# neozenith/sqlite-muninn

Measured on AMD Instinct MI355X. Metric: kNN queries/sec (10k-query batch, k=10, ef=128, 1M x 768 f32 HNSW index) + recall@10, higher is better.
Workload: dtype f32

## Files before the change

### sqlite-muninn_amd/csrc/mn_beam.hpp

```cpp
#pragma once
#include "mn_dist.hpp"

template <bool COH> DEVI int ld_link(const int *p) {
    if (COH)
        return __hip_atomic_load(p, __ATOMIC_RELAXED, __HIP_MEMORY_SCOPE_AGENT);
    return *p;
}
DEVI void st_link(int *p, int v) { __hip_atomic_store(p, v, __ATOMIC_RELAXED, __HIP_MEMORY_SCOPE_AGENT); }


struct WHeap {
    uint2 *l;
    unsigned long long *g;
    int lcap, gcap;
    int size;
    int ovf;
    int sorted = 0;
};

DEVI uint2 hget(const WHeap &h, int i) {
    if (i < h.lcap)
        return h.l[i];
    unsigned long long v = __hip_atomic_load(&h.g[i - h.lcap], __ATOMIC_RELAXED, __HIP_MEMORY_SCOPE_AGENT);
    return make_uint2((unsigned)(v & 0xffffffffull), (unsigned)(v >> 32));
}
DEVI void hset(const WHeap &h, int i, uint2 v) {
    if (i < h.lcap)
        h.l[i] = v;
    else
        __hip_atomic_store(&h.g[i - h.lcap], (unsigned long long)v.x | ((unsigned long long)v.y << 32), __ATOMIC_RELAXED,
                           __HIP_MEMORY_SCOPE_AGENT);
}

DEVI void heap_push(WHeap &h, int slot, float d, int lane) {
    if (h.size + 1 >= h.lcap + h.gcap) {
        h.ovf = 1;
        return;
    }
    h.size++;
    const int idx = h.size;
    const int depth = 31 - __clz(idx);
    const bool anc = lane >= 1 && lane <= depth;
    const int p = anc ? (idx >> lane) : idx;
    const uint2 x = make_uint2(f2u(d), (unsigned)slot);
    uint2 it = x;
    if (anc)
        it = hget(h, p);
    unsigned long long stopm = __ballot(anc && (u2f(it.x) <= d));
    const int stop = stopm ? (__ffsll((long long)stopm) - 1) : depth + 1;
    if (lane >= 1 && lane < stop)
        hset(h, idx >> (lane - 1), it);
    if (lane == 0)
        hset(h, idx >> (stop - 1), x);
    __builtin_amdgcn_wave_barrier();
}

DEVI uint2 heap_pop(WHeap &h, int lane) {
    uint2 top = hget(h, 1);
    top.x = rflu(top.x);
    top.y = rflu(top.y);
    uint2 x = hget(h, h.size);
    x.x = rflu(x.x);
    x.y = rflu(x.y);
    h.size--;
    if (h.size > 0) {
        int idx = 1;
        const float xd = u2f(x.x);
        for (;;) {
            int left = 2 * idx;
            if (left > h.size)
                break;
            uint2 L, Rt;
            if (left + 1 < h.lcap) {
                uint4 c = *reinterpret_cast<const uint4 *>(&h.l[left]);
                L = make_uint2(c.x, c.y);
                Rt = make_uint2(c.z, c.w);
            } else {
                L = hget(h, left);
                Rt = (left + 1 <= h.size) ? hget(h, left + 1) : L;
            }
            L.x = rflu(L.x);
            L.y = rflu(L.y);
            Rt.x = rflu(Rt.x);
            Rt.y = rflu(Rt.y);
            int smallest = idx;
            float sd = xd;
            uint2 sv = x;
            if (u2f(L.x) < sd) {
                smallest = left;
                sd = u2f(L.x);
                sv = L;
            }
            if (left + 1 <= h.size && u2f(Rt.x) < sd) {
                smallest = left + 1;
                sv = Rt;
            }
            if (smallest == idx)
                break;
            if (lane == 0)
                hset(h, idx, sv);
            idx = smallest;
        }
        if (lane == 0)
            hset(h, idx, x);
    }
    __builtin_amdgcn_wave_barrier();
    return top;
}


struct CoopCtx {
    int *n;
    int *list;
    float *dist;
    float *qnorm;
    int nw, wv;
    float *tile = nullptr;
    int tile_rows = 0;
};

#define MN_PHASE_N 16
#ifdef MN_PHASE_TIMING
static __device__ unsigned long long mn_phase[MN_PHASE_N];
#define PH_DECL unsigned long long ph_t = __builtin_amdgcn_s_memrealtime()
#define PH_ADD(w, k)                                                                                                             \
    do {                                                                                                                         \
        const unsigned long long ph_n = __builtin_amdgcn_s_memrealtime();                                                        \
        (w).ph[k] += ph_n - ph_t;                                                                                                \
        ph_t = ph_n;                                                                                                             \
// ... 650 lines not shown
```

### sqlite-muninn_amd/csrc/mn_device.hpp

```cpp
#pragma once
#include <hip/hip_runtime.h>
#include <stdint.h>
#include <stdlib.h>

#define MN_WAVE 64

typedef unsigned mn_lo_t;
#define MN_LO_BITS 10
#define MN_LO_CMAX 511
#define MN_LO_LINE_CODES 96
#define MN_LO_LINE_WORDS 32
struct __align__(16) MnLoMeta {
    float scale;
    float resid;
    float xn_lo;
    float xn_hi;
};
#define MN_LO_MIN_LD 192
__host__ __device__ inline bool mn_lo_enabled(int ld) { return ld >= MN_LO_MIN_LD && (ld & 63) == 0; }
__host__ __device__ inline int mn_lo_lines(int ld) { return (ld + MN_LO_LINE_CODES - 1) / MN_LO_LINE_CODES; }
__host__ __device__ inline size_t mn_lo_row_words(int ld) { return (size_t)mn_lo_lines(ld) * MN_LO_LINE_WORDS; }
__host__ __device__ inline int mn_lo_q_floats(int ld) { return mn_lo_enabled(ld) ? mn_lo_lines(ld) * MN_LO_LINE_CODES : ld; }
__host__ __device__ inline int mn_lo_code(unsigned w, int f) { return (int)(w << (32 - MN_LO_BITS * (f + 1))) >> (32 - MN_LO_BITS); }
__host__ __device__ inline unsigned mn_lo_pack(int c0, int c1, int c2) {
    return ((unsigned)c0 & 0x3ffu) | (((unsigned)c1 & 0x3ffu) << 10) | (((unsigned)c2 & 0x3ffu) << 20);
}
constexpr int MN_ORDER_SSE_V = 0;
constexpr int MN_ORDER_WAVE_V = 1;

struct MnDevIndex {
    const float *vectors;
    const float *norms;
    int *links0;
    int *links_up;
    const int *up_off;
    const signed char *levels;
    const unsigned char *deleted;
    unsigned char *dirty;
    const long long *ids;
    int dim, ld, metric, order;
    int W0, WU;
    int M0, MU;
    int WX;
    int n_slots;
    int n_pool_rows;
    int has_deleted;
    const mn_lo_t *vec_lo;
    const MnLoMeta *lo_meta;
};

#define MN_QC 6
struct MnSearchArgs {
    const float *queries;
    const int *query_slots;
    long long nq;
    int k;
    int ef;
    int entry_slot, max_level;
    long long *out_ids;
    float *out_dists;
    int *out_counts;
    int *sel;
    int *nsel;
    int nlev;
    const int *up_bm_index;
    unsigned *bitmap0;
    long long bm0_words;
    unsigned *bitmap_up;
    long long bmu_words;
    uint2 *cand_ovf;
    int cand_gcap;
    uint2 *res_ovf;
    int res_gcap;
    unsigned long long *counters;
    unsigned long long *q_counters;
    int use_tile;
    int lds_bitmap;
    int *readlog;
    int readcap;
    int *nread;
    int lat_tile_rows;
    unsigned lat_tile_off;
    int surv_lanes;
    int no_spec_rows;
};
size_t mn_lds_optin_limit();
bool mn_lds_grant(const void *kernel, size_t bytes);
template <typename K> inline bool mn_lds_grant_for(K kernel, size_t bytes) { return mn_lds_grant(reinterpret_cast<const void *>(kernel), bytes); }
inline int mn_no_spec_rows(long long n_slots, int ld) {
    const char *sr = getenv("MN_SPEC_ROWS");
    const bool big = (size_t)n_slots * ld * sizeof(float) > ((size_t)256 << 20);
    return sr ? (atoi(sr) == 0 ? 1 : 0) : (big ? 0 : 1);
}

#ifndef MN_CAND_LDS
#define MN_CAND_LDS 256
#endif
#ifndef MN_RES_LDS
#define MN_RES_LDS 256
#endif

void mn_module_touch_kernels();
void mn_module_touch_seq();
void mn_module_touch_spec();
void mn_module_touch_build();
void mn_launch_prep_rows(const MnDevIndex &ix, int first_slot, int n, float *norms_out, mn_lo_t *lo_out, MnLoMeta *meta_out,
                         hipStream_t st);
int mn_launch_dist_batch(int metric, int order, const float *d_query, const float *d_rows, long long n, int dim, int ld,
                         float *d_out, hipStream_t st);
size_t mn_dist_batch_lds_bytes(int ld);
size_t mn_search_lds_bytes(int ld, bool tile);
size_t mn_coop_lds_bytes(int ld, bool tile);
size_t mn_spec_commit_min_lds_bytes(int ld);
size_t mn_link_reverse_lds_bytes(int ld, int WX, int nq);
size_t mn_bruteforce_lds_bytes(int ld);
inline size_t mn_row_lds_bytes(int ld) { return (size_t)ld * sizeof(float); }
int mn_launch_search(const MnDevIndex &ix, const MnSearchArgs &a, bool build, hipStream_t st);
void mn_launch_bruteforce(const MnDevIndex &ix, const float *d_queries, long long nq, int k, long long *d_out_ids,
                          float *d_scratch, hipStream_t st);

size_t mn_brute_mfma_scratch_bytes(const MnDevIndex &ix, long long nq, int k, int *n_chunks_out, int *rows_per_chunk_out);
int mn_launch_bruteforce_mfma(const MnDevIndex &ix, const float *d_queries, long long nq, int k, long long *d_out_ids,
                              void *scratch, hipStream_t st);

struct MnExactSelf {
    int s0;
    float r;
    void *d_xc;
};
size_t mn_exact_mfma_scratch_bytes(const MnDevIndex &ix, long long nq, int kp, bool self = false);
int mn_launch_exact_mfma(const MnDevIndex &ix, const float *d_queries, long long nq, int k, int kp, const unsigned *d_allow,
                         void *scratch, long long *d_out_ids, float *d_out_d, int *d_out_cnt, unsigned long long *d_ctr,
                         int *d_marked, const MnExactSelf *self, hipStream_t st);
size_t mn_exact_valu_lds_bytes(int ld);
int mn_launch_exact_valu(const MnDevIndex &ix, const float *d_queries, const int *d_qsel, long long n, int k, const unsigned *d_allow,
                         long long *d_out_ids, float *d_out_d, int *d_out_cnt, const MnExactSelf *self, hipStream_t st);
void mn_launch_exact_fill(long long nq, int k, long long *d_out_ids, float *d_out_d, int *d_out_cnt, hipStream_t st);
void mn_launch_knn_prep_rows(const MnDevIndex &ix, void *d_xc, hipStream_t st);

int mn_index_search_overflow(struct mn_index *x, long long *n_overflow);
void mn_launch_merge_topk(const long long *g_ids, const float *g_dists, const int *g_counts, int world, long long nq, int k,
                          long long *out_ids, float *out_dists, int *out_counts, hipStream_t st);

struct MnLinkArgs {
    int level, M_max;
    int nq, nlev;
    const int *query_slots;
    const int *sel;
    const int *nsel;
    int *t_target;
    int *t_src;
    int *counters;
    int *count;
    int *fill;
    int *binoff;
    int *touched;
    int *bins;
    int *newrows;
    int world, rank;
    int *rec_count;
    int *records;
    int *cls_count;
};
void mn_launch_link(const MnDevIndex &ix, const MnLinkArgs &a, int max_tuples, hipStream_t st);
// ... 23 lines not shown
```

### sqlite-muninn_amd/csrc/mn_dist.hpp

```cpp
#pragma once
#include "mn_device.hpp"

#define DEVI __device__ __forceinline__

DEVI int rfl(int v) { return __builtin_amdgcn_readfirstlane(v); }
DEVI unsigned rflu(unsigned v) { return (unsigned)__builtin_amdgcn_readfirstlane((int)v); }
DEVI float u2f(unsigned u) { return __uint_as_float(u); }
DEVI unsigned f2u(float f) { return __float_as_uint(f); }
DEVI double rfl_f64(double v) {
    const unsigned long long b = (unsigned long long)__double_as_longlong(v);
    return __longlong_as_double((long long)(((unsigned long long)rflu((unsigned)(b >> 32)) << 32) | rflu((unsigned)b)));
}


DEVI float cosine_finish(float dot, float na, float nb) {
    float denom = __fmul_rn(sqrtf(na), sqrtf(nb));
    if (denom < 1e-30f)
        return 1.0f;
    return __fsub_rn(1.0f, __fdiv_rn(dot, denom));
}

DEVI float wave_butterfly(float acc) {
#pragma unroll
    for (int m = 32; m >= 1; m >>= 1)
// ... 571 lines not shown
            int s = __builtin_amdgcn_readlane(myslot, src);
            const float4 *row = reinterpret_cast<const float4 *>(ix.vectors + (size_t)s * ix.ld);
#pragma unroll
            for (int k = 0; k < NC; k++) {
                int e4 = k * 64 + lane;
                v[r][k] = (e4 * 4 < ix.ld) ? row[e4] : make_float4(0.f, 0.f, 0.f, 0.f);
            }
        }
#pragma unroll
        for (int r = 0; r < R; r++) {
            float acc = 0.0f;
#pragma unroll
            for (int k = 0; k < NC; k++) {
                int e4 = k * 64 + lane;
                if (e4 * 4 < ix.ld) {
                    float4 q = reinterpret_cast<const float4 *>(q_lds)[e4];
                    float4 b = v[r][k];
                    if (L2) {
                        float d0 = __fsub_rn(q.x, b.x), d1 = __fsub_rn(q.y, b.y), d2 = __fsub_rn(q.z, b.z),
                              d3 = __fsub_rn(q.w, b.w);
                        acc = fmaf(d0, d0, acc);
                        acc = fmaf(d1, d1, acc);
                        acc = fmaf(d2, d2, acc);
                        acc = fmaf(d3, d3, acc);
                    } else {
                        acc = fmaf(q.x, b.x, acc);
                        acc = fmaf(q.y, b.y, acc);
                        acc = fmaf(q.z, b.z, acc);
                        acc = fmaf(q.w, b.w, acc);
                    }
                }
            }
            acc = wave_butterfly(acc);
            if (lane == t + r)
                mine = acc;
        }
    }
    return mine;
}

template <int ORDER, int NCH, bool LAT = false>
DEVI float rows_distance(const MnDevIndex &ix, const float *q_lds, float qnorm, int myslot, int n, int lane,
                         float *tile = nullptr, int tile_rows = 0) {
    if (ix.metric == 0) {
        return rows_accumulate<ORDER, NCH, true, LAT>(ix, q_lds, myslot, n, lane, tile, tile_rows);
    }
    float dot = rows_accumulate<ORDER, NCH, false, LAT>(ix, q_lds, myslot, n, lane, tile, tile_rows);
    if (ix.metric == 2)
        return -dot;
    float nb = (lane < n) ? ix.norms[myslot] : 1.0f;
    return cosine_finish(dot, qnorm, nb);
}

DEVI float rows_distance_spread(const MnDevIndex &ix, const float *q_lds, float qnorm, int myslot, int n, int lane, int Q) {
    if (ix.metric == 0)
        return sse_rows_spread<true>(ix, q_lds, myslot, n, lane, Q);
    const float dot = sse_rows_spread<false>(ix, q_lds, myslot, n, lane, Q);
    if (ix.metric == 2)
        return -dot;
    const float nb = (lane < n) ? ix.norms[myslot] : 1.0f;
    return cosine_finish(dot, qnorm, nb);
}


DEVI float lo_deq(int c, float s) { return __fmul_rn((float)c, s); }
DEVI double mn_gamma(int n) {
    const double nu = (double)n * 0x1p-24;
    return nu / (1.0 - nu);
}

template <bool L2, int UB>
DEVI void lo_lines(const uint4 *__restrict__ row, const float *q, float s, int lines, int &k, float &acc) {
    for (; k + UB <= lines; k += UB) {
        uint4 v[UB];
#pragma unroll
        for (int u = 0; u < UB; u++)
            v[u] = row[8 * (k + u)];
        __builtin_amdgcn_sched_barrier(0);
#pragma unroll
        for (int u = 0; u < UB; u++) {
            const float4 qa = *reinterpret_cast<const float4 *>(q + MN_LO_LINE_CODES * (k + u));
            const float4 qb = *reinterpret_cast<const float4 *>(q + MN_LO_LINE_CODES * (k + u) + 4);
            const float4 qc = *reinterpret_cast<const float4 *>(q + MN_LO_LINE_CODES * (k + u) + 8);
            const float qe[12] = {qa.x, qa.y, qa.z, qa.w, qb.x, qb.y, qb.z, qb.w, qc.x, qc.y, qc.z, qc.w};
            const unsigned w4[4] = {v[u].x, v[u].y, v[u].z, v[u].w};
#pragma unroll
            for (int e = 0; e < 12; e++) {
                const float x = lo_deq(mn_lo_code(w4[e / 3], e % 3), s);
                if (L2) {
                    const float d = __fsub_rn(qe[e], x);
                    acc = fmaf(d, d, acc);
                } else {
                    acc = fmaf(qe[e], x, acc);
                }
            }
            __builtin_amdgcn_sched_barrier(0);
        }
    }
}

template <bool L2>
DEVI float lo_rows_accumulate(const MnDevIndex &ix, const float *q_lds, int myslot, float sc, int n, int lane) {
    float mine = 0.0f;
    int ln = lane;
    asm volatile("" : "+v"(ln));
    const int c = ln & 7, r = ln >> 3;
    const int lines = mn_lo_lines(ix.ld);
    const size_t row_words = mn_lo_row_words(ix.ld);
    for (int t = 0; t < n; t += 8) {
        const int rr = t + r < n ? t + r : n - 1;
        const int sl = __shfl(myslot, rr);
        const float s = __shfl(sc, rr);
        const uint4 *row = reinterpret_cast<const uint4 *>(ix.vec_lo + (size_t)sl * row_words) + c;
        const float *q = q_lds + 12 * c;
        float acc = 0.0f;
        int k = 0;
        lo_lines<L2, 8>(row, q, s, lines, k, acc);
        lo_lines<L2, 2>(row, q, s, lines, k, acc);
        lo_lines<L2, 1>(row, q, s, lines, k, acc);
        acc += quad_xor1(acc);
        acc += quad_xor2(acc);
        acc += __int_as_float(__builtin_amdgcn_ds_swizzle(__float_as_int(acc), 0x101F));
        const float got = __shfl(acc, ((ln - t) & 7) << 3);
        if (ln >= t && ln < t + 8)
            mine = got;
    }
    return mine;
}

struct LoQuery {
    double qs_lo;
    double qn_hi;
};
DEVI LoQuery lo_query(float qsq, int ld) {
    LoQuery lq;
    lq.qs_lo = sqrt((double)qsq) * (1.0 - 0x1p-40);
    const double lost = (double)ld * 0x1p-149;
    lq.qn_hi = sqrt(((double)qsq + lost) / (1.0 - 2.0 * mn_gamma(ld + 8))) * (1.0 + 0x1p-40);
    return lq;
}

DEVI float lo_lower_bound(int metric, float A, const MnLoMeta &m, const LoQuery &lq, int ld) {
    const double a = A, r = m.resid, g = mn_gamma(ld + 8), u = 0x1p-24;
    if (!(fabs(a) <= 3.0e38) || !(r <= 3.0e38))
        return -__builtin_inff();
    double lb;
    if (metric == 0) {
        const double l = (double)sqrtf((float)(fmax(a - (double)ld * 0x1p-147, 0.0) * (1.0 - 4.0 * g))) * (1.0 - 0x1p-21) - 2.0 * r;
        lb = l > 0.0 ? l * l * (1.0 - 4.0 * g) : 0.0;
    } else {
        const double e = 2.0 * (lq.qn_hi * (r + g * (2.0 * (double)m.xn_hi + r)) + (double)ld * 0x1p-147);
        if (metric == 2) {
            lb = -(a + e);
        } else {
            const double den = lq.qs_lo * (double)m.xn_lo * (1.0 - 8.0 * u);
            if (!(den >= 1e-28))
                return -__builtin_inff();
            lb = 1.0 - fmax(a + e, 0.0) / den * (1.0 + 4.0 * u);
        }
    }
    lb -= fabs(lb) * 0x1p-20 + 0x1p-120;
    const float f = __double2float_rd(lb);
    return f == f ? f : -__builtin_inff();
}

template <int ORDER>
DEVI float lds_self_norm(const float *q_lds, int dim, int ld, int lane) {
    if (ORDER == MN_ORDER_SSE_V) {
        float v = sse_row<false>(q_lds, q_lds, dim, lane);
        return __shfl(v, 0);
    }
    return wave_row_generic<false>(q_lds, q_lds, ld, lane);
}

DEVI float lo_rows_bound(const MnDevIndex &ix, const float *q_lds, const LoQuery &lq, int myslot, int n, int lane) {
    MnLoMeta m = {1.0f, __builtin_inff(), 0.0f, 0.0f};
    if (lane < n)
        m = ix.lo_meta[myslot];
    const float A = ix.metric == 0 ? lo_rows_accumulate<true>(ix, q_lds, myslot, m.scale, n, lane)
                                   : lo_rows_accumulate<false>(ix, q_lds, myslot, m.scale, n, lane);
    return lane < n ? lo_lower_bound(ix.metric, A, m, lq, ix.ld) : -__builtin_inff();
}
```

### sqlite-muninn_amd/csrc/mn_kernels.hip

```cpp
#include "mn_device.hpp"
#include <cstdio>
#include <cstdlib>
#include <mutex>
#include <unordered_map>

#include "mn_dist.hpp"
#include "mn_dispatch.hpp"


DEVI double wave_sum_f64(double v) {
#pragma unroll
    for (int m = 32; m >= 1; m >>= 1)
        v += __shfl_xor(v, m);
    return v;
}

template <int ORDER>
__global__ void __launch_bounds__(64)
    k_prep_rows(MnDevIndex ix, int first_slot, int n, float *norms_out, mn_lo_t *lo_out, MnLoMeta *meta_out) {
    extern __shared__ float lds[];
    const int lane = threadIdx.x;
    int slot = first_slot + blockIdx.x;
    if (blockIdx.x >= n)
        return;
    const float *row = ix.vectors + (size_t)slot * ix.ld;
    for (int i = lane; i < ix.ld; i += 64)
        lds[i] = row[i];
    __builtin_amdgcn_s_waitcnt(0);
    __builtin_amdgcn_wave_barrier();
    float nbv = 0.0f;
    if (norms_out) {
        nbv = lds_self_norm<ORDER>(lds, ix.dim, ix.ld, lane);
        if (lane == 0)
            norms_out[slot] = nbv;
    }
    if (!lo_out)
        return;
    float mx = 0.0f;
    bool bad = false;
    for (int i = lane; i < ix.ld; i += 64) {
        const float v = lds[i];
        bad |= !(fabsf(v) <= 3.4028235e38f);
        mx = fmaxf(mx, fabsf(v));
    }
    for (int m = 32; m >= 1; m >>= 1)
        mx = fmaxf(mx, __shfl_xor(mx, m));
    bad = __ballot(bad) != 0;
    float s = __fdiv_rn(mx, (float)MN_LO_CMAX);
    bad |= !(s >= 1.17549435e-38f && s <= 3.4028235e38f);
    if (bad)
        s = 0.0f;
    double r2 = 0.0, x2 = 0.0;
    mn_lo_t *lo = lo_out + (size_t)slot * mn_lo_row_words(ix.ld);
    const int words = (int)mn_lo_row_words(ix.ld);
    for (int w = lane; w < words; w += 64) {
        int c[3];
#pragma unroll
        for (int f = 0; f < 3; f++) {
            const int i = 3 * w + f;
            c[f] = 0;
            if (i < ix.ld) {
                const float v = lds[i];
                if (!bad) {
                    const float t = rintf(__fdiv_rn(v, s));
                    c[f] = (int)fminf(fmaxf(t, -(float)MN_LO_CMAX), (float)MN_LO_CMAX);
                }
                const double dv = (double)v - (double)lo_deq(c[f], s);
                r2 += dv * dv;
                x2 += (double)v * (double)v;
            }
        }
        lo[w] = mn_lo_pack(c[0], c[1], c[2]);
    }
    r2 = wave_sum_f64(r2);
    x2 = wave_sum_f64(x2);
    if (lane == 0) {
        MnLoMeta m;
        m.scale = s;
        const double xn = sqrt(x2), rx = sqrt(r2);
        m.xn_lo = norms_out ? __double2float_rd(sqrt((double)nbv) * (1.0 - 0x1p-40)) : __double2float_rd(xn * (1.0 - 0x1p-36));
        m.xn_hi = __double2float_ru(xn * (1.0 + 0x1p-36));
        m.resid = __double2float_ru(rx * (1.0 + 0x1p-36) + 0x1p-140);
        if (bad || !(m.xn_hi <= 3.0e38f) || !(m.resid <= 3.0e38f))
            m.resid = __builtin_inff();
        meta_out[slot] = m;
    }
}

void mn_launch_prep_rows(const MnDevIndex &ix, int first_slot, int n, float *norms_out, mn_lo_t *lo_out, MnLoMeta *meta_out,
                         hipStream_t st) {
    if (n <= 0 || (!norms_out && !lo_out))
        return;
    size_t lds = mn_row_lds_bytes(ix.ld);
    if (ix.order == MN_ORDER_SSE_V)
        hipLaunchKernelGGL(k_prep_rows<MN_ORDER_SSE_V>, dim3(n), dim3(64), lds, st, ix, first_slot, n, norms_out, lo_out, meta_out);
    else
        hipLaunchKernelGGL(k_prep_rows<MN_ORDER_WAVE_V>, dim3(n), dim3(64), lds, st, ix, first_slot, n, norms_out, lo_out, meta_out);
}


template <int ORDER, int NCH>
__global__ void __launch_bounds__(64)
    k_dist_batch(int metric, const float *query, const float *rows, long long n, int dim, int ld, float *out) {
    extern __shared__ float lds[];
    const int lane = threadIdx.x;
    for (int i = lane; i < ld; i += 64)
        lds[i] = i < dim ? query[i] : 0.0f;
    __builtin_amdgcn_s_waitcnt(0);
    __builtin_amdgcn_wave_barrier();
    MnDevIndex ix = {};
    ix.vectors = rows;
    ix.dim = dim;
    ix.ld = ld;
    ix.metric = metric;
    float qnorm = 0.0f;
    if (metric == 1)
        qnorm = lds_self_norm<ORDER>(lds, dim, ld, lane);
    long long base = (long long)blockIdx.x * 64;
    int cnt = (int)((n - base) < 64 ? (n - base) : 64);
    if (cnt <= 0)
        return;
    ix.vectors = rows + (size_t)base * ld;
    int myslot = lane < cnt ? lane : 0;
    float d;
    if (metric == 0) {
        d = rows_accumulate<ORDER, NCH, true>(ix, lds, myslot, cnt, lane);
    } else {
        float dot = rows_accumulate<ORDER, NCH, false>(ix, lds, myslot, cnt, lane);
        if (metric == 2) {
            d = -dot;
        } else {
            float nb = 0.0f;
            for (int t = 0; t < cnt; t++) {
                const float *row = ix.vectors + (size_t)t * ld;
                float *tmp = lds + ld;
                for (int i = lane; i < ld; i += 64)
                    tmp[i] = row[i];
                __builtin_amdgcn_s_waitcnt(0);
                __builtin_amdgcn_wave_barrier();
                float v = lds_self_norm<ORDER>(tmp, dim, ld, lane);
                __builtin_amdgcn_wave_barrier();
                if (lane == t)
                    nb = v;
            }
            d = cosine_finish(dot, qnorm, nb);
        }
    }
    if (lane < cnt)
        out[base + lane] = d;
}

size_t mn_dist_batch_lds_bytes(int ld) { return (size_t)ld * sizeof(float) * 2; }

template <int ORDER, int NCH>
static int launch_dist_batch(int metric, const float *d_query, const float *d_rows, long long n, int dim, int ld, float *d_out,
                             hipStream_t st) {
    const size_t lds = mn_dist_batch_lds_bytes(ld);
    if (lds > mn_lds_optin_limit() || !mn_lds_grant_for(k_dist_batch<ORDER, NCH>, lds))
        return -1;
    hipLaunchKernelGGL((k_dist_batch<ORDER, NCH>), dim3((unsigned)((n + 63) / 64)), dim3(64), lds, st, metric, d_query, d_rows, n,
                       dim, ld, d_out);
    return hipGetLastError() == hipSuccess ? 0 : -1;
}

int mn_launch_dist_batch(int metric, int order, const float *d_query, const float *d_rows, long long n, int dim, int ld,
                         float *d_out, hipStream_t st) {
    if (n <= 0)
        return 0;
    return mn_for_row_walk(order, ld, [&](auto O, auto N) {
        return launch_dist_batch<O(), N()>(metric, d_query, d_rows, n, dim, ld, d_out, st);
    });
}

#include "mn_beam.hpp"

template <int ORDER, int NCH, bool BUILD, bool WIDE, bool LAT = false, bool LP = false>
DEVI void beam_query(const MnDevIndex &ix, const MnSearchArgs &a, const long long qi, const int lane, unsigned char *smem,
                     CoopCtx *coop, unsigned *lds_bitmap = nullptr) {
    uint2 *cand_l = reinterpret_cast<uint2 *>(smem);
    uint2 *res_l = cand_l + MN_CAND_LDS;
    int *scratch = reinterpret_cast<int *>(res_l + MN_RES_LDS);
    float *q = reinterpret_cast<float *>(scratch + 64);
    const int qf = mn_lo_q_floats(ix.ld);
    float *tile = q + qf;

    int qslot = -1;
    const float *qsrc;
    if (BUILD) {
        qslot = a.query_slots[qi];
        qsrc = ix.vectors + (size_t)qslot * ix.ld;
    } else {
        qsrc = a.queries + (size_t)qi * ix.dim;
    }
    for (int i = lane; i < qf; i += 64)
        q[i] = i < ix.dim ? qsrc[i] : 0.0f;
    __builtin_amdgcn_s_waitcnt(0);
    __builtin_amdgcn_wave_barrier();

    WaveCtx w;
    w.q = q;
    w.tile = (ORDER == MN_ORDER_SSE_V && a.use_tile) ? tile : nullptr;
    w.scratch = scratch;
    w.n_dist = 0;
    w.n_exp = 0;
    w.qnorm = 0.0f;
    if (ix.metric == 1)
        w.qnorm = BUILD ? ix.norms[qslot] : lds_self_norm<ORDER>(q, ix.dim, ix.ld, lane);
    if (coop) {
        w.coop = coop;
        w.no_spec_rows = a.no_spec_rows;
        if (lane == 0)
            *coop->qnorm = w.qnorm;
    }
    if (LP) {
        w.lq = lo_query(ix.metric == 1 ? w.qnorm : lds_self_norm<ORDER>(q, ix.dim, ix.ld, lane), ix.ld);
        w.lp_on = w.lq.qn_hi <= 1.0e300;
        w.lq.qs_lo = rfl_f64(w.lq.qs_lo);
        w.lq.qn_hi = rfl_f64(w.lq.qn_hi);
        w.qnorm = u2f(rflu(f2u(w.qnorm)));
        w.sv_lanes = a.surv_lanes;
    }
    if (BUILD && a.readlog) {
        w.rlog = a.readlog + (size_t)qi * a.readcap * MN_RLOG_INTS;
        w.rcap = a.readcap;
    }

    WHeap cand, res;
    cand.l = cand_l;
    cand.lcap = MN_CAND_LDS;
    cand.g = reinterpret_cast<unsigned long long *>(a.cand_ovf + (size_t)qi * a.cand_gcap);
    cand.gcap = a.cand_gcap;
    cand.size = 0;
    cand.ovf = 0;
    res.l = res_l;
    res.lcap = MN_RES_LDS;
    res.g = reinterpret_cast<unsigned long long *>(a.res_ovf + (size_t)qi * a.res_gcap);
    res.gcap = a.res_gcap;
    res.size = 0;
    res.ovf = 0;

    unsigned *bm0 = lds_bitmap ? lds_bitmap : a.bitmap0 + (size_t)qi * a.bm0_words;
    int cur = a.entry_slot;

    if (!BUILD) {
        for (int l = a.max_level; l > 0; l--)
            cur = greedy_layer<ORDER, NCH, false, WIDE>(ix, w, cur, l, lane);
        if (LAT)
            beam_layer_auto<ORDER, NCH, false, WIDE>(ix, w, cand, res, bm0, a.bm0_words, cur, 0, a.ef, lane);
        else
            beam_layer<ORDER, NCH, false, WIDE, false, LP>(ix, w, cand, res, bm0, cur, 0, a.ef, lane);
        int count = res.size;
        int outn = count < a.k ? count : a.k;
        for (int i = count - 1; i >= 0; i--) {
            uint2 it = res_take(res, i, count, lane);
            if (i < a.k && lane == 0) {
                a.out_ids[qi * a.k + i] = ix.ids[it.y];
                a.out_dists[qi * a.k + i] = -u2f(it.x);
            }
        }
        if (lane == 0) {
            for (int i = outn; i < a.k; i++) {
                a.out_ids[qi * a.k + i] = -1;
                a.out_dists[qi * a.k + i] = 0.0f;
            }
            a.out_counts[qi] = outn;
        }
    } else {
        const int level = ix.levels[qslot];
        for (int l = a.max_level; l > level; l--)
            cur = greedy_layer<ORDER, NCH, false, WIDE, LAT>(ix, w, cur, l, lane);
        int start = level < a.max_level ? level : a.max_level;
        for (int l = start; l >= 0; l--) {
            unsigned *bm = bm0;
            if (l > 0)
                bm = a.bitmap_up + ((size_t)a.up_bm_index[qi] * a.max_level + (l - 1)) * a.bmu_words;
            if (LAT)
                beam_layer_auto<ORDER, NCH, false, WIDE, true>(ix, w, cand, res, bm, l > 0 ? a.bmu_words : a.bm0_words, cur, l, a.ef, lane);
            else
                beam_layer<ORDER, NCH, false, WIDE>(ix, w, cand, res, bm, cur, l, a.ef, lane);
            const int M_max = (l == 0) ? ix.M0 : ix.MU;
            int count = res.size;
            int keep = count < M_max ? count : M_max;
            int *sel = a.sel + ((size_t)qi * a.nlev + l) * ix.M0;
            int first = cur;
            for (int i = count - 1; i >= 0; i--) {
                uint2 it = res_take(res, i, count, lane);
                if (i < keep && lane == 0)
                    sel[i] = (int)it.y;
// ... 25 lines not shown
                atomicAdd(&a.counters[3], w.n_skip);
            if (LP && w.n_l8)
                atomicAdd(&a.counters[4], w.n_l8);
            if (LP && w.n_l16)
                atomicAdd(&a.counters[5], w.n_l16);
        }
    }
}

template <int ORDER, int NCH, bool BUILD, bool WIDE = false, bool LP = false>
__global__ void __launch_bounds__(64) k_beam(MnDevIndex ix, MnSearchArgs a) {
    extern __shared__ __align__(16) unsigned char smem[];
    if ((long long)blockIdx.x >= a.nq)
        return;
    beam_query<ORDER, NCH, BUILD, WIDE, false, LP>(ix, a, blockIdx.x, threadIdx.x, smem, nullptr);
}

#define MN_COOP_WAVES 8
template <int ORDER, int NCH, bool BUILD, bool WIDE = false>
__global__ void __launch_bounds__(MN_COOP_WAVES * 64) k_beam_coop(MnDevIndex ix, MnSearchArgs a, size_t base_lds) {
    extern __shared__ __align__(16) unsigned char smem[];
    if ((long long)blockIdx.x >= a.nq)
        return;
    const int lane = threadIdx.x & 63;
    CoopCtx c;
    c.n = reinterpret_cast<int *>(smem + base_lds);
    c.qnorm = reinterpret_cast<float *>(c.n + 1);
    c.list = c.n + 4;
    c.dist = reinterpret_cast<float *>(c.list + 64);
    c.nw = blockDim.x >> 6;
    c.wv = threadIdx.x >> 6;
    if (a.lat_tile_rows > 0) {
        c.tile = reinterpret_cast<float *>(smem + a.lat_tile_off) + (size_t)c.wv * mn_lat_tile_floats(ix.ld, a.lat_tile_rows);
        c.tile_rows = a.lat_tile_rows;
    }
    unsigned *lbm = nullptr;
    if (!BUILD && a.lds_bitmap) {
        lbm = reinterpret_cast<unsigned *>(smem + base_lds) + 4 + 64 + 64;
        for (long long i = threadIdx.x; i < a.bm0_words; i += blockDim.x)
            lbm[i] = 0u;
        __syncthreads();
    }
    if (c.wv == 0) {
        beam_query<ORDER, NCH, BUILD, WIDE, true>(ix, a, blockIdx.x, lane, smem, &c, lbm);
        if (lane == 0)
            *c.n = -1;
        __syncthreads();
    } else {
        const float *q = reinterpret_cast<const float *>(smem + (size_t)(MN_CAND_LDS + MN_RES_LDS) * sizeof(uint2) + 64 * sizeof(int));
        coop_helper<ORDER, NCH>(ix, q, c, lane);
    }
}

size_t mn_search_lds_bytes(int ld, bool tile) {
    size_t b = (size_t)(MN_CAND_LDS + MN_RES_LDS) * sizeof(uint2) + 64 * sizeof(int) + (size_t)mn_lo_q_floats(ld) * sizeof(float);
    if (tile)
        b += MN_TILE_FLOATS * sizeof(float);
    if (const char *pad = getenv("MN_LDS_PAD_BYTES"))
        b += (size_t)atoi(pad);
    return b;
}
size_t mn_coop_lds_bytes(int ld, bool tile) { return ((mn_search_lds_bytes(ld, tile) + 15) & ~(size_t)15) + (4 + 64 + 64) * sizeof(int); }

size_t mn_lds_optin_limit() {
    static std::mutex mu;
    static std::unordered_map<int, size_t> lims;
    int dev = 0;
    (void)hipGetDevice(&dev);
    std::lock_guard<std::mutex> lk(mu);
    auto it = lims.find(dev);
    if (it != lims.end())
        return it->second;
    size_t lim = 64 * 1024;
    const char *e = getenv("MN_LDS_OPTIN");
    int v = 0;
    if (!(e && atoi(e) == 0) && hipDeviceGetAttribute(&v, hipDeviceAttributeSharedMemPerBlockOptin, dev) == hipSuccess && v > 64 * 1024)
        lim = (size_t)v;
    (void)hipGetLastError();
    lims[dev] = lim;
    return lim;
}
bool mn_lds_grant(const void *kern, size_t bytes) {
    if (bytes <= 64 * 1024)
        return true;
    static std::mutex mu;
    struct Seen {
        size_t granted = 0;
        size_t refused = (size_t)-1;
    };
    static std::unordered_map<unsigned long long, Seen> seen;
    int dev = 0;
    (void)hipGetDevice(&dev);
    const unsigned long long key = (unsigned long long)reinterpret_cast<uintptr_t>(kern) * 64ull + (unsigned)(dev & 63);
    std::lock_guard<std::mutex> lk(mu);
    Seen &sn = seen[key];
    if (sn.granted >= bytes)
        return true;
    if (bytes >= sn.refused)
        return false;
    const bool ok = hipFuncSetAttribute(kern, hipFuncAttributeMaxDynamicSharedMemorySize, (int)bytes) == hipSuccess;
    if (ok) {
        sn.granted = bytes;
    } else {
        (void)hipGetLastError();
        sn.refused = bytes;
    }
    return ok;
}

template <int ORDER, int NCH, bool BUILD, bool WIDE>
static void launch_coop(const MnDevIndex &ix, MnSearchArgs a, size_t base, size_t tot, hipStream_t st) {
    const char *te = getenv("MN_LAT_TILE");
    if (ORDER == MN_ORDER_SSE_V && ix.ld >= 256 && !(te && atoi(te) == 0)) {
        const size_t off = (tot + 15) & ~(size_t)15;
        for (int rows = 4; rows >= 2; rows >>= 1) {
            const size_t need = off + (size_t)MN_COOP_WAVES * mn_lat_tile_floats(ix.ld, rows) * sizeof(float);
            if (need <= mn_lds_optin_limit() && mn_lds_grant_for(k_beam_coop<ORDER, NCH, BUILD, WIDE>, need)) {
                a.lat_tile_rows = rows;
                a.lat_tile_off = (unsigned)off;
                tot = need;
                break;
            }
        }
    }
    if (getenv("MN_LAT_DEBUG"))
        fprintf(stderr, "[mn] k_beam_coop: distance tile of %d rows per wavefront, %zu bytes of LDS\n", a.lat_tile_rows, tot);
    hipLaunchKernelGGL((k_beam_coop<ORDER, NCH, BUILD, WIDE>), dim3((unsigned)a.nq), dim3(MN_COOP_WAVES * 64), tot, st, ix, a, base);
}

template <int ORDER, int NCH>
static void launch_beam(const MnDevIndex &ix, const MnSearchArgs &a, bool build, hipStream_t st) {
    dim3 grid((unsigned)a.nq), block(64);
    size_t lds = mn_search_lds_bytes(ix.ld, ORDER == MN_ORDER_SSE_V && a.use_tile);
    const bool wide = ix.WX > 64;
    const char *co = getenv("MN_COOP");
    if (a.nq <= 128 && !(co && atoi(co) == 0)) {
        const size_t base = (lds + 15) & ~(size_t)15;
        const size_t tot = mn_coop_lds_bytes(ix.ld, ORDER == MN_ORDER_SSE_V && a.use_tile) +
                           (!build && a.lds_bitmap ? (size_t)a.bm0_words * sizeof(unsigned) : 0);
        if (wide) {
            if (build)
                launch_coop<ORDER, NCH, true, true>(ix, a, base, tot, st);
            else
                launch_coop<ORDER, NCH, false, true>(ix, a, base, tot, st);
        } else if (build)
            launch_coop<ORDER, NCH, true, false>(ix, a, base, tot, st);
        else
            launch_coop<ORDER, NCH, false, false>(ix, a, base, tot, st);
        return;
    }
    const char *lp = getenv("MN_LOWPREC_FILTER");
    if (!build && ix.vec_lo && ix.lo_meta && !(lp && atoi(lp) == 0)) {
        MnSearchArgs al = a;
        const char *sv = getenv("MN_SURVIVOR_LANES");
        const int svl = sv ? atoi(sv) : 0;
        al.surv_lanes = (svl == 4 || svl == 8 || svl == 16) ? svl : 0;
        if (wide)
            hipLaunchKernelGGL((k_beam<ORDER, NCH, false, true, true>), grid, block, lds, st, ix, al);
        else
            hipLaunchKernelGGL((k_beam<ORDER, NCH, false, false, true>), grid, block, lds, st, ix, al);
        return;
    }
    if (wide) {
        if (build)
            hipLaunchKernelGGL((k_beam<ORDER, NCH, true, true>), grid, block, lds, st, ix, a);
        else
            hipLaunchKernelGGL((k_beam<ORDER, NCH, false, true>), grid, block, lds, st, ix, a);
    } else if (build)
        hipLaunchKernelGGL((k_beam<ORDER, NCH, true>), grid, block, lds, st, ix, a);
    else
        hipLaunchKernelGGL((k_beam<ORDER, NCH, false>), grid, block, lds, st, ix, a);
}

int mn_launch_search(const MnDevIndex &ix, const MnSearchArgs &a, bool build, hipStream_t st) {
    if (a.nq <= 0)
        return 0;
    if (ix.order == MN_ORDER_SSE_V) {
        const char *qe = getenv("MN_SSE_QUAD");
        if (MN_SSE_QUAD2 > 0 && (ix.dim >> 4) >= MN_SSE_QUAD2 && !(qe && atoi(qe) == 0))
            launch_beam<MN_ORDER_SSE_V, 1>(ix, a, build, st);
        else
            launch_beam<MN_ORDER_SSE_V, 0>(ix, a, build, st);
        return 0;
    }
    mn_for_wave_walk(ix.ld, [&](auto O, auto N) { launch_beam<O(), N()>(ix, a, build, st); });
    return 0;
}


template <int ORDER, int NCH>
__global__ void __launch_bounds__(64)
    k_edge_rows(MnDevIndex ix, const int *row_slot, const int *row_level, int n_rows, int *out_nbr, float *out_dist) {
    extern __shared__ __align__(16) unsigned char smem[];
    const int lane = threadIdx.x;
    const int r = blockIdx.x;
    if (r >= n_rows)
        return;
    float *q = reinterpret_cast<float *>(smem);
    const int s = row_slot[r], level = row_level[r];
    const float *sv = ix.vectors + (size_t)s * ix.ld;
    for (int i = lane; i < ix.ld; i += 64)
        q[i] = sv[i];
    __builtin_amdgcn_s_waitcnt(0);
    __builtin_amdgcn_wave_barrier();
    int W;
    const int *row = link_row(ix, s, level, W);
    for (int c0 = 0; c0 < ix.WX; c0 += 64) {
        const int p = c0 + lane;
        const int nb = p < W ? row[p] : -1;
        const int n = __popcll(__ballot(nb >= 0));
        float d = 0.0f;
        if (n > 0) {
            const int myslot = lane < n ? nb : 0;
            d = rows_distance<ORDER, NCH>(ix, q, ix.metric == 1 ? ix.norms[s] : 0.0f, myslot, n, lane);
            if (lane < n && ix.deleted[myslot])
                d = 0.0f;
        }
        if (p < ix.WX) {
            out_nbr[(size_t)r * ix.WX + p] = nb;
            out_dist[(size_t)r * ix.WX + p] = d;
        }
    }
}

// ... 71 lines not shown
```

Before: 594,600.

## Size LDS heaps to the occupancy budget and prefetch row metadata earlier

The beam-search kernel now picks the sizes of the LDS-resident candidate and result heaps at launch time. It queries occupancy so that extra LDS is used only where it costs no wavefronts per CU: the result heap is shrunk to about ef and the candidate heap grows into the slack, which should reduce spills to the global overflow heap. Heap pop also loads both spilled children from global memory together instead of one at a time. Norm and low-precision metadata loads are issued before the distance accumulation so their latency overlaps it. The risks are added host-side occupancy queries and a mismatch between the chosen LDS layout and what the kernel expects.

```diff
diff --git a/sqlite-muninn_amd/csrc/mn_beam.hpp b/sqlite-muninn_amd/csrc/mn_beam.hpp
--- a/sqlite-muninn_amd/csrc/mn_beam.hpp
+++ b/sqlite-muninn_amd/csrc/mn_beam.hpp
@@ -55,11 +55,14 @@
     __builtin_amdgcn_wave_barrier();
 }
 
+#ifndef MN_SPILL_PAIR
+#define MN_SPILL_PAIR 1
+#endif
 DEVI uint2 heap_pop(WHeap &h, int lane) {
     uint2 top = hget(h, 1);
+    uint2 x = hget(h, h.size);
     top.x = rflu(top.x);
     top.y = rflu(top.y);
-    uint2 x = hget(h, h.size);
     x.x = rflu(x.x);
     x.y = rflu(x.y);
     h.size--;
@@ -75,6 +78,13 @@
                 uint4 c = *reinterpret_cast<const uint4 *>(&h.l[left]);
                 L = make_uint2(c.x, c.y);
                 Rt = make_uint2(c.z, c.w);
+            } else if (MN_SPILL_PAIR && left >= h.lcap) {
+                const unsigned long long *gp = &h.g[left - h.lcap];
+                const int ro = (left + 1 <= h.size) ? 1 : 0;
+                const unsigned long long lv = __hip_atomic_load(gp, __ATOMIC_RELAXED, __HIP_MEMORY_SCOPE_AGENT);
+                const unsigned long long rv = __hip_atomic_load(gp + ro, __ATOMIC_RELAXED, __HIP_MEMORY_SCOPE_AGENT);
+                L = make_uint2((unsigned)(lv & 0xffffffffull), (unsigned)(lv >> 32));
+                Rt = make_uint2((unsigned)(rv & 0xffffffffull), (unsigned)(rv >> 32));
             } else {
                 L = hget(h, left);
                 Rt = (left + 1 <= h.size) ? hget(h, left + 1) : L;
diff --git a/sqlite-muninn_amd/csrc/mn_device.hpp b/sqlite-muninn_amd/csrc/mn_device.hpp
--- a/sqlite-muninn_amd/csrc/mn_device.hpp
+++ b/sqlite-muninn_amd/csrc/mn_device.hpp
@@ -83,6 +83,7 @@
     unsigned lat_tile_off;
     int surv_lanes;
     int no_spec_rows;
+    int cand_lcap, res_lcap;
 };
 size_t mn_lds_optin_limit();
 bool mn_lds_grant(const void *kernel, size_t bytes);
@@ -109,7 +110,7 @@
 int mn_launch_dist_batch(int metric, int order, const float *d_query, const float *d_rows, long long n, int dim, int ld,
                          float *d_out, hipStream_t st);
 size_t mn_dist_batch_lds_bytes(int ld);
-size_t mn_search_lds_bytes(int ld, bool tile);
+size_t mn_search_lds_bytes(int ld, bool tile, int cand_lcap = MN_CAND_LDS, int res_lcap = MN_RES_LDS);
 size_t mn_coop_lds_bytes(int ld, bool tile);
 size_t mn_spec_commit_min_lds_bytes(int ld);
 size_t mn_link_reverse_lds_bytes(int ld, int WX, int nq);
diff --git a/sqlite-muninn_amd/csrc/mn_dist.hpp b/sqlite-muninn_amd/csrc/mn_dist.hpp
--- a/sqlite-muninn_amd/csrc/mn_dist.hpp
+++ b/sqlite-muninn_amd/csrc/mn_dist.hpp
@@ -647,13 +647,20 @@
     return cosine_finish(dot, qnorm, nb);
 }
 
+#ifndef MN_META_AHEAD
+#define MN_META_AHEAD 1
+#endif
 DEVI float rows_distance_spread(const MnDevIndex &ix, const float *q_lds, float qnorm, int myslot, int n, int lane, int Q) {
     if (ix.metric == 0)
         return sse_rows_spread<true>(ix, q_lds, myslot, n, lane, Q);
+    float nb = 1.0f;
+    if (MN_META_AHEAD && ix.metric == 1 && lane < n)
+        nb = ix.norms[myslot];
     const float dot = sse_rows_spread<false>(ix, q_lds, myslot, n, lane, Q);
     if (ix.metric == 2)
         return -dot;
-    const float nb = (lane < n) ? ix.norms[myslot] : 1.0f;
+    if (!MN_META_AHEAD && lane < n)
+        nb = ix.norms[myslot];
     return cosine_finish(dot, qnorm, nb);
 }
 
@@ -665,13 +672,20 @@
 }
 
 template <bool L2, int UB>
-DEVI void lo_lines(const uint4 *__restrict__ row, const float *q, float s, int lines, int &k, float &acc) {
+DEVI void lo_lines(const uint4 *__restrict__ row, const float *q, float sc, int rr, int lines, int &k, float &acc) {
+    float s = 0.0f;
+    if (!MN_META_AHEAD)
+        s = __shfl(sc, rr);
     for (; k + UB <= lines; k += UB) {
         uint4 v[UB];
 #pragma unroll
         for (int u = 0; u < UB; u++)
             v[u] = row[8 * (k + u)];
         __builtin_amdgcn_sched_barrier(0);
+        if (MN_META_AHEAD) {
+            asm volatile("" : "+v"(rr));
+            s = __shfl(sc, rr);
+        }
 #pragma unroll
         for (int u = 0; u < UB; u++) {
             const float4 qa = *reinterpret_cast<const float4 *>(q + MN_LO_LINE_CODES * (k + u));
@@ -705,14 +719,13 @@
     for (int t = 0; t < n; t += 8) {
         const int rr = t + r < n ? t + r : n - 1;
         const int sl = __shfl(myslot, rr);
-        const float s = __shfl(sc, rr);
         const uint4 *row = reinterpret_cast<const uint4 *>(ix.vec_lo + (size_t)sl * row_words) + c;
         const float *q = q_lds + 12 * c;
         float acc = 0.0f;
         int k = 0;
-        lo_lines<L2, 8>(row, q, s, lines, k, acc);
-        lo_lines<L2, 2>(row, q, s, lines, k, acc);
-        lo_lines<L2, 1>(row, q, s, lines, k, acc);
+        lo_lines<L2, 8>(row, q, sc, rr, lines, k, acc);
+        lo_lines<L2, 2>(row, q, sc, rr, lines, k, acc);
+        lo_lines<L2, 1>(row, q, sc, rr, lines, k, acc);
         acc += quad_xor1(acc);
         acc += quad_xor2(acc);
         acc += __int_as_float(__builtin_amdgcn_ds_swizzle(__float_as_int(acc), 0x101F));
@@ -770,7 +783,9 @@
 
 DEVI float lo_rows_bound(const MnDevIndex &ix, const float *q_lds, const LoQuery &lq, int myslot, int n, int lane) {
     MnLoMeta m = {1.0f, __builtin_inff(), 0.0f, 0.0f};
-    if (lane < n)
+    if (MN_META_AHEAD)
+        m = ix.lo_meta[lane < n ? myslot : 0];
+    else if (lane < n)
         m = ix.lo_meta[myslot];
     const float A = ix.metric == 0 ? lo_rows_accumulate<true>(ix, q_lds, myslot, m.scale, n, lane)
                                    : lo_rows_accumulate<false>(ix, q_lds, myslot, m.scale, n, lane);
diff --git a/sqlite-muninn_amd/csrc/mn_kernels.hip b/sqlite-muninn_amd/csrc/mn_kernels.hip
--- a/sqlite-muninn_amd/csrc/mn_kernels.hip
+++ b/sqlite-muninn_amd/csrc/mn_kernels.hip
@@ -1,6 +1,8 @@
 #include "mn_device.hpp"
+#include <atomic>
 #include <cstdio>
 #include <cstdlib>
+#include <initializer_list>
 #include <mutex>
 #include <unordered_map>
 
@@ -177,9 +179,11 @@
 template <int ORDER, int NCH, bool BUILD, bool WIDE, bool LAT = false, bool LP = false>
 DEVI void beam_query(const MnDevIndex &ix, const MnSearchArgs &a, const long long qi, const int lane, unsigned char *smem,
                      CoopCtx *coop, unsigned *lds_bitmap = nullptr) {
+    const int cand_lcap = (!LAT && a.cand_lcap) ? a.cand_lcap : MN_CAND_LDS;
+    const int res_lcap = (!LAT && a.cand_lcap) ? a.res_lcap : MN_RES_LDS;
     uint2 *cand_l = reinterpret_cast<uint2 *>(smem);
-    uint2 *res_l = cand_l + MN_CAND_LDS;
-    int *scratch = reinterpret_cast<int *>(res_l + MN_RES_LDS);
+    uint2 *res_l = cand_l + cand_lcap;
+    int *scratch = reinterpret_cast<int *>(res_l + res_lcap);
     float *q = reinterpret_cast<float *>(scratch + 64);
     const int qf = mn_lo_q_floats(ix.ld);
     float *tile = q + qf;
@@ -227,13 +231,13 @@
 
     WHeap cand, res;
     cand.l = cand_l;
-    cand.lcap = MN_CAND_LDS;
+    cand.lcap = cand_lcap;
     cand.g = reinterpret_cast<unsigned long long *>(a.cand_ovf + (size_t)qi * a.cand_gcap);
     cand.gcap = a.cand_gcap;
     cand.size = 0;
     cand.ovf = 0;
     res.l = res_l;
-    res.lcap = MN_RES_LDS;
+    res.lcap = res_lcap;
     res.g = reinterpret_cast<unsigned long long *>(a.res_ovf + (size_t)qi * a.res_gcap);
     res.gcap = a.res_gcap;
     res.size = 0;
@@ -365,8 +369,8 @@
     }
 }
 
-size_t mn_search_lds_bytes(int ld, bool tile) {
-    size_t b = (size_t)(MN_CAND_LDS + MN_RES_LDS) * sizeof(uint2) + 64 * sizeof(int) + (size_t)mn_lo_q_floats(ld) * sizeof(float);
+size_t mn_search_lds_bytes(int ld, bool tile, int cand_lcap, int res_lcap) {
+    size_t b = (size_t)(cand_lcap + res_lcap) * sizeof(uint2) + 64 * sizeof(int) + (size_t)mn_lo_q_floats(ld) * sizeof(float);
     if (tile)
         b += MN_TILE_FLOATS * sizeof(float);
     if (const char *pad = getenv("MN_LDS_PAD_BYTES"))
@@ -441,15 +445,87 @@
     hipLaunchKernelGGL((k_beam_coop<ORDER, NCH, BUILD, WIDE>), dim3((unsigned)a.nq), dim3(MN_COOP_WAVES * 64), tot, st, ix, a, base);
 }
 
+#ifndef MN_HEAP_CARVE
+#define MN_HEAP_CARVE 1
+#endif
+static int beam_lds_budget(const void *kern) {
+    static std::mutex mu;
+    static std::unordered_map<unsigned long long, int> seen;
+    int dev = 0;
+    (void)hipGetDevice(&dev);
+    const unsigned long long key = (unsigned long long)reinterpret_cast<uintptr_t>(kern) * 64ull + (unsigned)(dev & 63);
+    std::lock_guard<std::mutex> lk(mu);
+    auto it = seen.find(key);
+    if (it != seen.end())
+        return it->second;
+    int budget = 0, r0 = 0, cu_lds = 0;
+    hipFuncAttributes fa;
+    if (hipOccupancyMaxActiveBlocksPerMultiprocessor(&r0, kern, 64, 0) == hipSuccess && r0 > 0 &&
+        hipDeviceGetAttribute(&cu_lds, hipDeviceAttributeMaxSharedMemoryPerMultiprocessor, dev) == hipSuccess && cu_lds > 0 &&
+        hipFuncGetAttributes(&fa, kern) == hipSuccess) {
+        for (const int gran : {256, 1280, 2560}) {
+            const int b = cu_lds / r0 / gran * gran - (int)fa.sharedSizeBytes;
+            int r1 = 0;
+            if (b > 0 && b <= 64 * 1024 && hipOccupancyMaxActiveBlocksPerMultiprocessor(&r1, kern, 64, (size_t)b) == hipSuccess &&
+                r1 == r0) {
+                budget = b;
+                break;
+            }
+        }
+    }
+    (void)hipGetLastError();
+    if (getenv("MN_LAT_DEBUG"))
+        fprintf(stderr, "[mn] k_beam %p: %d wavefronts per CU by registers, %d bytes of LDS per CU, %d per wavefront\n", kern, r0,
+                cu_lds, budget);
+    seen[key] = budget;
+    return budget;
+}
+static size_t beam_carve(const void *kern, int ld, bool tile, MnSearchArgs &a) {
+    a.cand_lcap = MN_CAND_LDS;
+    a.res_lcap = MN_RES_LDS;
+    const int budget = MN_HEAP_CARVE ? beam_lds_budget(kern) : 0;
+    const char *fe = getenv("MN_CAND_LDS_ENTRIES");
+    if (MN_HEAP_CARVE && (budget > 0 || fe)) {
+        a.res_lcap = a.ef < 255 ? ((a.ef + 3) & ~1) : MN_RES_LDS;
+        const long long rest = (long long)budget - (long long)mn_search_lds_bytes(ld, tile, 0, a.res_lcap);
+        long long c = rest > 0 ? rest / (long long)sizeof(uint2) : 0;
+        if (fe)
+            c = atoll(fe) < 2 ? 2 : atoll(fe);
+        else if (c < MN_CAND_LDS)
+            c = MN_CAND_LDS;
+        const long long most = ((long long)MN_LDS_LIMIT - (long long)mn_search_lds_bytes(ld, tile, 0, a.res_lcap)) / (long long)sizeof(uint2);
+        if (c > most)
+            c = most;
+        a.cand_lcap = (int)(c & ~1ll);
+        if (a.cand_lcap < 2) {
+            a.cand_lcap = MN_CAND_LDS;
+            a.res_lcap = MN_RES_LDS;
+        }
+    }
+    const size_t lds = mn_search_lds_bytes(ld, tile, a.cand_lcap, a.res_lcap);
+    if (getenv("MN_LAT_DEBUG")) {
+        static std::atomic<unsigned long long> last{0};
+        const unsigned long long sig = ((unsigned long long)a.cand_lcap << 40) ^ ((unsigned long long)a.res_lcap << 20) ^ (unsigned long long)lds;
+        if (last.exchange(sig) != sig)
+            fprintf(stderr, "[mn] k_beam: ld %d ef %d: candidate heap %d entries in LDS, results %d, %zu bytes of LDS\n", ld, a.ef,
+                    a.cand_lcap, a.res_lcap, lds);
+    }
+    return lds;
+}
+template <typename K> static void launch_k_beam(K kern, const MnDevIndex &ix, MnSearchArgs a, bool tile, hipStream_t st) {
+    const size_t lds = beam_carve(reinterpret_cast<const void *>(kern), ix.ld, tile, a);
+    hipLaunchKernelGGL(kern, dim3((unsigned)a.nq), dim3(64), lds, st, ix, a);
+}
+
 template <int ORDER, int NCH>
 static void launch_beam(const MnDevIndex &ix, const MnSearchArgs &a, bool build, hipStream_t st) {
-    dim3 grid((unsigned)a.nq), block(64);
-    size_t lds = mn_search_lds_bytes(ix.ld, ORDER == MN_ORDER_SSE_V && a.use_tile);
+    const bool tile = ORDER == MN_ORDER_SSE_V && a.use_tile;
+    size_t lds = mn_search_lds_bytes(ix.ld, tile);
     const bool wide = ix.WX > 64;
     const char *co = getenv("MN_COOP");
     if (a.nq <= 128 && !(co && atoi(co) == 0)) {
         const size_t base = (lds + 15) & ~(size_t)15;
-        const size_t tot = mn_coop_lds_bytes(ix.ld, ORDER == MN_ORDER_SSE_V && a.use_tile) +
+        const size_t tot = mn_coop_lds_bytes(ix.ld, tile) +
                            (!build && a.lds_bitmap ? (size_t)a.bm0_words * sizeof(unsigned) : 0);
         if (wide) {
             if (build)
@@ -469,20 +545,20 @@
         const int svl = sv ? atoi(sv) : 0;
         al.surv_lanes = (svl == 4 || svl == 8 || svl == 16) ? svl : 0;
         if (wide)
-            hipLaunchKernelGGL((k_beam<ORDER, NCH, false, true, true>), grid, block, lds, st, ix, al);
+            launch_k_beam(k_beam<ORDER, NCH, false, true, true>, ix, al, tile, st);
         else
-            hipLaunchKernelGGL((k_beam<ORDER, NCH, false, false, true>), grid, block, lds, st, ix, al);
+            launch_k_beam(k_beam<ORDER, NCH, false, false, true>, ix, al, tile, st);
         return;
     }
     if (wide) {
         if (build)
-            hipLaunchKernelGGL((k_beam<ORDER, NCH, true, true>), grid, block, lds, st, ix, a);
+            launch_k_beam(k_beam<ORDER, NCH, true, true>, ix, a, tile, st);
         else
-            hipLaunchKernelGGL((k_beam<ORDER, NCH, false, true>), grid, block, lds, st, ix, a);
+            launch_k_beam(k_beam<ORDER, NCH, false, true>, ix, a, tile, st);
     } else if (build)
-        hipLaunchKernelGGL((k_beam<ORDER, NCH, true>), grid, block, lds, st, ix, a);
+        launch_k_beam(k_beam<ORDER, NCH, true>, ix, a, tile, st);
     else
-        hipLaunchKernelGGL((k_beam<ORDER, NCH, false>), grid, block, lds, st, ix, a);
+        launch_k_beam(k_beam<ORDER, NCH, false>, ix, a, tile, st);
 }
 
 int mn_launch_search(const MnDevIndex &ix, const MnSearchArgs &a, bool build, hipStream_t st) {
```

Result: faster. 608,300, median of 6 (+2.3%).

## Embed per-row quantization metadata in spare code bits for inner-product bounds

Applied to the files above, without the earlier changes.

Packs the 16-byte per-row metadata (scale, residual, norm bounds) into the unused top 2 bits of the first 64 code dwords of each 10-bit quantized row. For non-L2 metrics the kernel then rebuilds the metadata from the code lines it already loads, so the separate lo_meta gather goes away. It also accumulates raw integer codes and applies the scale once at the end. In exchange it adds shuffle work to reassemble the metadata, widens the residual and error bounds slightly to cover the changed rounding, and leaves the L2 path unchanged.

```diff
diff --git a/sqlite-muninn_amd/csrc/mn_device.hpp b/sqlite-muninn_amd/csrc/mn_device.hpp
--- a/sqlite-muninn_amd/csrc/mn_device.hpp
+++ b/sqlite-muninn_amd/csrc/mn_device.hpp
@@ -24,6 +24,20 @@
 __host__ __device__ inline int mn_lo_code(unsigned w, int f) { return (int)(w << (32 - MN_LO_BITS * (f + 1))) >> (32 - MN_LO_BITS); }
 __host__ __device__ inline unsigned mn_lo_pack(int c0, int c1, int c2) {
     return ((unsigned)c0 & 0x3ffu) | (((unsigned)c1 & 0x3ffu) << 10) | (((unsigned)c2 & 0x3ffu) << 20);
+}
+__host__ __device__ inline unsigned mn_lo_meta_put(unsigned code_dword, int w, const unsigned m[4]) {
+    const int c = (w & 31) >> 2, p = 4 * (w >> 5) + (w & 3);
+    return code_dword | (((m[c >> 1] >> (16 * (c & 1) + 14 - 2 * p)) & 3u) << 30);
+}
+__host__ __device__ inline unsigned mn_lo_meta_share(const unsigned l0[4], const unsigned l1[4]) {
+    unsigned h = 0;
+#pragma unroll
+    for (int j = 0; j < 4; j++)
+        h = (h << 2) | (l0[j] >> 30);
+#pragma unroll
+    for (int j = 0; j < 4; j++)
+        h = (h << 2) | (l1[j] >> 30);
+    return h;
 }
 constexpr int MN_ORDER_SSE_V = 0;
 constexpr int MN_ORDER_WAVE_V = 1;
diff --git a/sqlite-muninn_amd/csrc/mn_dist.hpp b/sqlite-muninn_amd/csrc/mn_dist.hpp
--- a/sqlite-muninn_amd/csrc/mn_dist.hpp
+++ b/sqlite-muninn_amd/csrc/mn_dist.hpp
@@ -664,14 +664,20 @@
     return nu / (1.0 - nu);
 }
 
-template <bool L2, int UB>
-DEVI void lo_lines(const uint4 *__restrict__ row, const float *q, float s, int lines, int &k, float &acc) {
+template <bool L2, int UB, bool META = false>
+DEVI void lo_lines(const uint4 *__restrict__ row, const float *q, float s, int lines, int &k, float &acc, unsigned *share = nullptr) {
     for (; k + UB <= lines; k += UB) {
         uint4 v[UB];
 #pragma unroll
         for (int u = 0; u < UB; u++)
             v[u] = row[8 * (k + u)];
         __builtin_amdgcn_sched_barrier(0);
+        if constexpr (META && UB >= 2) {
+            if (k == 0) {
+                const unsigned l0[4] = {v[0].x, v[0].y, v[0].z, v[0].w}, l1[4] = {v[1].x, v[1].y, v[1].z, v[1].w};
+                *share = mn_lo_meta_share(l0, l1);
+            }
+        }
 #pragma unroll
         for (int u = 0; u < UB; u++) {
             const float4 qa = *reinterpret_cast<const float4 *>(q + MN_LO_LINE_CODES * (k + u));
@@ -681,12 +687,12 @@
             const unsigned w4[4] = {v[u].x, v[u].y, v[u].z, v[u].w};
 #pragma unroll
             for (int e = 0; e < 12; e++) {
-                const float x = lo_deq(mn_lo_code(w4[e / 3], e % 3), s);
+                const int code = mn_lo_code(w4[e / 3], e % 3);
                 if (L2) {
-                    const float d = __fsub_rn(qe[e], x);
+                    const float d = __fsub_rn(qe[e], lo_deq(code, s));
                     acc = fmaf(d, d, acc);
                 } else {
-                    acc = fmaf(qe[e], x, acc);
+                    acc = fmaf(qe[e], (float)code, acc);
                 }
             }
             __builtin_amdgcn_sched_barrier(0);
@@ -695,7 +701,7 @@
 }
 
 template <bool L2>
-DEVI float lo_rows_accumulate(const MnDevIndex &ix, const float *q_lds, int myslot, float sc, int n, int lane) {
+DEVI float lo_rows_accumulate(const MnDevIndex &ix, const float *q_lds, int myslot, MnLoMeta &m, int n, int lane) {
     float mine = 0.0f;
     int ln = lane;
     asm volatile("" : "+v"(ln));
@@ -705,20 +711,37 @@
     for (int t = 0; t < n; t += 8) {
         const int rr = t + r < n ? t + r : n - 1;
         const int sl = __shfl(myslot, rr);
-        const float s = __shfl(sc, rr);
+        const float s = L2 ? __shfl(m.scale, rr) : 0.0f;
         const uint4 *row = reinterpret_cast<const uint4 *>(ix.vec_lo + (size_t)sl * row_words) + c;
         const float *q = q_lds + 12 * c;
         float acc = 0.0f;
+        unsigned share = 0;
         int k = 0;
-        lo_lines<L2, 8>(row, q, s, lines, k, acc);
-        lo_lines<L2, 2>(row, q, s, lines, k, acc);
+        lo_lines<L2, 8, !L2>(row, q, s, lines, k, acc, &share);
+        lo_lines<L2, 2, !L2>(row, q, s, lines, k, acc, &share);
         lo_lines<L2, 1>(row, q, s, lines, k, acc);
         acc += quad_xor1(acc);
         acc += quad_xor2(acc);
         acc += __int_as_float(__builtin_amdgcn_ds_swizzle(__float_as_int(acc), 0x101F));
-        const float got = __shfl(acc, ((ln - t) & 7) << 3);
-        if (ln >= t && ln < t + 8)
-            mine = got;
+        const int src = ((ln - t) & 7) << 3;
+        const float got = __shfl(acc, src);
+        const bool take = ln >= t && ln < t + 8;
+        if (L2) {
+            if (take)
+                mine = got;
+        } else {
+            const unsigned other = (unsigned)__float_as_int(quad_xor1(__int_as_float((int)share)));
+            const unsigned word = (c & 1) ? (other | (share << 16)) : (share | (other << 16));
+            const unsigned w0 = (unsigned)__shfl((int)word, src), w1 = (unsigned)__shfl((int)word, src + 2);
+            const unsigned w2 = (unsigned)__shfl((int)word, src + 4), w3 = (unsigned)__shfl((int)word, src + 6);
+            if (take) {
+                m.scale = __uint_as_float(w0);
+                m.resid = __uint_as_float(w1);
+                m.xn_lo = __uint_as_float(w2);
+                m.xn_hi = __uint_as_float(w3);
+                mine = __fmul_rn(m.scale, got);
+            }
+        }
     }
     return mine;
 }
@@ -744,7 +767,7 @@
         const double l = (double)sqrtf((float)(fmax(a - (double)ld * 0x1p-147, 0.0) * (1.0 - 4.0 * g))) * (1.0 - 0x1p-21) - 2.0 * r;
         lb = l > 0.0 ? l * l * (1.0 - 4.0 * g) : 0.0;
     } else {
-        const double e = 2.0 * (lq.qn_hi * (r + g * (2.0 * (double)m.xn_hi + r)) + (double)ld * 0x1p-147);
+        const double e = 2.0 * (lq.qn_hi * (r + g * (2.0 * (double)m.xn_hi + r)) + (double)ld * 0x1p-147 * fmax(1.0, (double)m.scale));
         if (metric == 2) {
             lb = -(a + e);
         } else {
@@ -770,9 +793,13 @@
 
 DEVI float lo_rows_bound(const MnDevIndex &ix, const float *q_lds, const LoQuery &lq, int myslot, int n, int lane) {
     MnLoMeta m = {1.0f, __builtin_inff(), 0.0f, 0.0f};
-    if (lane < n)
-        m = ix.lo_meta[myslot];
-    const float A = ix.metric == 0 ? lo_rows_accumulate<true>(ix, q_lds, myslot, m.scale, n, lane)
-                                   : lo_rows_accumulate<false>(ix, q_lds, myslot, m.scale, n, lane);
+    float A;
+    if (ix.metric == 0) {
+        if (lane < n)
+            m = ix.lo_meta[myslot];
+        A = lo_rows_accumulate<true>(ix, q_lds, myslot, m, n, lane);
+    } else {
+        A = lo_rows_accumulate<false>(ix, q_lds, myslot, m, n, lane);
+    }
     return lane < n ? lo_lower_bound(ix.metric, A, m, lq, ix.ld) : -__builtin_inff();
 }
diff --git a/sqlite-muninn_amd/csrc/mn_kernels.hip b/sqlite-muninn_amd/csrc/mn_kernels.hip
--- a/sqlite-muninn_amd/csrc/mn_kernels.hip
+++ b/sqlite-muninn_amd/csrc/mn_kernels.hip
@@ -53,6 +53,7 @@
     double r2 = 0.0, x2 = 0.0;
     mn_lo_t *lo = lo_out + (size_t)slot * mn_lo_row_words(ix.ld);
     const int words = (int)mn_lo_row_words(ix.ld);
+    unsigned first = 0;
     for (int w = lane; w < words; w += 64) {
         int c[3];
 #pragma unroll
@@ -65,26 +66,32 @@
                     const float t = rintf(__fdiv_rn(v, s));
                     c[f] = (int)fminf(fmaxf(t, -(float)MN_LO_CMAX), (float)MN_LO_CMAX);
                 }
-                const double dv = (double)v - (double)lo_deq(c[f], s);
+                const double dv = (double)v - (double)c[f] * (double)s;
                 r2 += dv * dv;
                 x2 += (double)v * (double)v;
             }
         }
-        lo[w] = mn_lo_pack(c[0], c[1], c[2]);
+        const unsigned pk = mn_lo_pack(c[0], c[1], c[2]);
+        if (w < 2 * MN_LO_LINE_WORDS)
+            first = pk;
+        else
+            lo[w] = pk;
     }
     r2 = wave_sum_f64(r2);
     x2 = wave_sum_f64(x2);
-    if (lane == 0) {
-        MnLoMeta m;
-        m.scale = s;
-        const double xn = sqrt(x2), rx = sqrt(r2);
-        m.xn_lo = norms_out ? __double2float_rd(sqrt((double)nbv) * (1.0 - 0x1p-40)) : __double2float_rd(xn * (1.0 - 0x1p-36));
-        m.xn_hi = __double2float_ru(xn * (1.0 + 0x1p-36));
-        m.resid = __double2float_ru(rx * (1.0 + 0x1p-36) + 0x1p-140);
-        if (bad || !(m.xn_hi <= 3.0e38f) || !(m.resid <= 3.0e38f))
-            m.resid = __builtin_inff();
+    MnLoMeta m;
+    m.scale = s;
+    const double xn = sqrt(x2), rx = sqrt(r2);
+    m.xn_lo = norms_out ? __double2float_rd(sqrt((double)nbv) * (1.0 - 0x1p-40)) : __double2float_rd(xn * (1.0 - 0x1p-36));
+    m.xn_hi = __double2float_ru(xn * (1.0 + 0x1p-36));
+    m.resid = __double2float_ru((rx + 0x1p-24 * (xn + rx)) * (1.0 + 0x1p-36) + 0x1p-140);
+    if (bad || !(m.xn_hi <= 3.0e38f) || !(m.resid <= 3.0e38f))
+        m.resid = __builtin_inff();
+    const unsigned mw[4] = {(unsigned)__shfl(__float_as_int(m.scale), 0), (unsigned)__shfl(__float_as_int(m.resid), 0),
+                            (unsigned)__shfl(__float_as_int(m.xn_lo), 0), (unsigned)__shfl(__float_as_int(m.xn_hi), 0)};
+    lo[lane] = mn_lo_meta_put(first, lane, mw);
+    if (lane == 0)
         meta_out[slot] = m;
-    }
 }
 
 void mn_launch_prep_rows(const MnDevIndex &ix, int first_slot, int n, float *norms_out, mn_lo_t *lo_out, MnLoMeta *meta_out,
```

Measured after the change: 598,100 before, 621,900 after, median of 6. 1.04x the previous value.
